# Clemapfel/kmer_index

Hardware: AMD Instinct MI355X
Metric: M queries/sec, DNA4 k=10 exact-match batch search, 1e8-bp text (higher is better)
Workload: dtype u32/u64

## Files before the change

kmer_index_amd/csrc/kmx_capi.hip:

```cpp
#include <hip/hip_runtime.h>

#include <algorithm>
#include <atomic>
#include <cstddef>
#include <cstdio>
#include <cstdlib>
#include <cstring>
#include <memory>
#include <mutex>
#include <string>
#include <system_error>
#include <thread>
#include <vector>

#include "kmx_approx.h"
#include "kmx_host.h"
#include "kmx_kernels.h"

namespace {

thread_local std::string g_err;

kmx_status fail(kmx_status st, const std::string& msg)
{
// ... 1331 lines not shown
    if (r && !r->parts.empty()) return fail(KMX_ERR_INVALID_ARGUMENT, "kmx_search_batch_device: the result handle belongs to a multi-device search");
    if (r && r->device != ix->device && r->device_bytes())
        return fail(KMX_ERR_INVALID_ARGUMENT, "kmx_search_batch_device: the result handle holds buffers on another device");
    if (!r) { r = take_result(ix); *inout = r; }
    else if (r->ctx.pending) { kmx_status fs = search_finish(r); if (fs != KMX_OK) return fs; }
    r->index = ix;
    r->device = ix->device;
    r->stream = s;
    (void)hipGetLastError();
    r->flags = flags;
    r->nq = nq;
    r->n_hits = r->n_exact = r->n_stitch = r->n_prefix = r->n_error = r->n_none = r->n_mask_words = 0;
    r->host_valid = r->host_masks_valid = false;
    r->small_valid = false;
    r->quiesced = false;
    if (!r->h_ctr) HIP_TRY(hipHostMalloc(reinterpret_cast<void**>(&r->h_ctr), KMX_CTR_COUNT * sizeof(unsigned long long), hipHostMallocDefault));
    HIP_TRY(r->hit_off.ensure((nq + 1) * 8));
    if (nq == 0) {
        HIP_TRY(hipMemsetAsync(r->hit_off.p, 0, 8, s));
        return KMX_OK;
    }
    HIP_TRY(r->src.ensure(nq * 8));
    HIP_TRY(r->cnt.ensure(nq * 4));
    HIP_TRY(r->c0.ensure(nq * 4));
    HIP_TRY(r->aux.ensure(nq * 8));
    HIP_TRY(r->key.ensure(nq * 8));
    HIP_TRY(r->p1.ensure(nq * 8));
    HIP_TRY(r->kind.ensure(nq));
    HIP_TRY(r->status.ensure(nq));
    HIP_TRY(r->stitch_list.ensure(nq * 4));
    HIP_TRY(r->prefix_list.ensure(nq * 4));
    HIP_TRY(r->short_list.ensure(nq * 4));
    HIP_TRY(r->bsum.ensure(std::max(kmx::scan_blocks(nq), kmx::lookup_blocks(nq, 4)) * 8));
    if (r->ctr.cap < 2 * KMX_CTR_COUNT * sizeof(unsigned long long)) {
        HIP_TRY(r->ctr.ensure(2 * KMX_CTR_COUNT * sizeof(unsigned long long)));
        HIP_TRY(hipMemsetAsync(r->ctr.p, 0, 2 * KMX_CTR_COUNT * sizeof(unsigned long long), s));
        r->ctr_phase = 0;
        r->ctr_clean = true;
    }
    kmx::QueryDesc d{r->src.as<uint64_t>(), r->cnt.as<uint32_t>(), r->c0.as<uint32_t>(), r->aux.as<uint64_t>(),
                     r->key.as<uint64_t>(), r->p1.as<uint64_t>(), r->kind.as<uint8_t>(), r->status.as<uint8_t>(),
                     r->stitch_list.as<uint32_t>(), r->prefix_list.as<uint32_t>(), r->short_list.as<uint32_t>(), nullptr};
    if (!r->ctr_clean) {
        HIP_TRY(hipMemsetAsync(r->ctr.p, 0, 2 * KMX_CTR_COUNT * sizeof(unsigned long long), s));
        r->ctr_clean = true;
    }
    r->ctr_phase ^= 1u;
    auto* ctr = r->ctr.as<unsigned long long>() + r->ctr_phase * KMX_CTR_COUNT;
    auto* ctr_next = r->ctr.as<unsigned long long>() + (r->ctr_phase ^ 1u) * KMX_CTR_COUNT;
    const KmxIndexDev* dix = header_for(ix, flags);

    static const int force_items = getenv("KMX_LOOKUP_ITEMS") ? atoi(getenv("KMX_LOOKUP_ITEMS")) : 0;
    const bool pairs = force_items ? force_items == -4 : r->last_had_pairs;
    const int items = force_items ? (force_items == 8 ? 8 : 4) : (!pairs && ix->tiny_cells) ? 8 : 4;
    const bool defer_long = r->last_had_long;
    const uint32_t lflags = (flags & ~KMX_SEARCH_INTERNAL_DEFER_LONG) | (defer_long ? KMX_SEARCH_INTERNAL_DEFER_LONG : 0u);
    timed(ix, K_LOOKUP, s, [&] {
        kmx::launch_lookup(s, items, pairs, dix, qr, qo, nq, d, ctr, r->bsum.as<uint64_t>(), lflags);
        if (defer_long) kmx::launch_lookup_long(s, dix, qr, qo, nq, d, ctr, flags);
    });
    const kmx::FillVariant fv = kmx::effective_fill_variant(ix->fill_variant, ix->rec32);
    const uint64_t tile = kmx::fill_tile(fv);
    const uint64_t tile_cap = r->tile_q.cap / 4;
    bool published = false;
    timed(ix, K_SCAN, s, [&] {
        published = kmx::launch_scan_tiles(s, d.cnt, nq, r->bsum.as<uint64_t>(), r->hit_off.as<uint64_t>(), ctr + KMX_CTR_TOTAL_HITS, tile,
                                           tile_cap >= 2 ? tile_cap - 1 : 0, tile_cap >= 2 ? r->tile_q.as<uint32_t>() : nullptr, items,
                                           kmx::CounterPub{ctr, ctr_next, r->h_ctr});
    });
    r->ctr_clean = published;
    const uint64_t spec_tiles = std::min<uint64_t>(tile_cap >= 2 ? tile_cap - 1 : 0, (r->out.cap / 4) / tile);
    const bool spec_fill = !(flags & KMX_SEARCH_COUNT_ONLY) && !r->last_had_stitch && spec_tiles > 0 && spec_tiles < 0x7FFFFFFFull;
    if (spec_fill)
        timed(ix, K_FILL, s, [&] {
            kmx::launch_fill(s, fv, ix->rec32, dix, ix->d_arena, r->hit_off.as<uint64_t>(), r->tile_q.as<uint32_t>(),
                             ctr + KMX_CTR_TOTAL_HITS, spec_tiles, d, r->out.as<uint32_t>());
        });
    if (!published) HIP_TRY(hipMemcpyAsync(r->h_ctr, ctr, KMX_CTR_COUNT * sizeof(unsigned long long), hipMemcpyDeviceToHost, s));
    r->ctx = SearchCtx{ix, qr, qo, s, tile_cap, spec_tiles, spec_fill, true};
    if (flags & KMX_SEARCH_ASYNC) {
        if (!r->done) HIP_TRY(hipEventCreateWithFlags(&r->done, hipEventDisableTiming));
        HIP_TRY(hipEventRecord(r->done, s));
        r->pool = ix->pool;
        std::lock_guard<std::mutex> lock(ix->pool->mu);
        ix->pool->pending.push_back(r);
        return KMX_OK;
    }
    return search_finish(r);
}

static kmx_status search_finish(kmx_result* r)
{
    if (!r->ctx.pending) return KMX_OK;
    r->ctx.pending = false;
    kmx_index* ix = r->ctx.ix;
    if (r->flags & KMX_SEARCH_ASYNC) {
        std::lock_guard<std::mutex> lock(ix->pool->mu);
        auto& pend = ix->pool->pending;
        pend.erase(std::remove(pend.begin(), pend.end(), r), pend.end());
    }
    const uint8_t* qr = r->ctx.qr;
// ... 1088 lines not shown
```

kmer_index_amd/csrc/kmx_kernels.h:

```cpp
#pragma once
#include <hip/hip_runtime.h>
#include <stdint.h>
#include "kmx_types.h"


namespace kmx {

struct QueryDesc {
    uint64_t* src;
    uint32_t* cnt;
    uint32_t* c0;
    uint64_t* aux;
    uint64_t* key;
    uint64_t* p1;
    uint8_t* kind;
    uint8_t* status;
    uint32_t* stitch_list;
    uint32_t* prefix_list;
    uint32_t* short_list;
    uint32_t* stitch_hits;
};

uint64_t lookup_blocks(uint64_t nq, int items);
void launch_lookup(hipStream_t s, int items, bool pairs, const KmxIndexDev* ix, const uint8_t* qranks, const uint64_t* qoff,
                   uint64_t nq, const QueryDesc& d, unsigned long long* ctr, uint64_t* block_hits, uint32_t flags);
void launch_lookup_long(hipStream_t s, const KmxIndexDev* ix, const uint8_t* qranks, const uint64_t* qoff, uint64_t nq, const QueryDesc& d,
                        unsigned long long* ctr, uint32_t flags);
void launch_validate(hipStream_t s, const KmxIndexDev* ix, const uint32_t* arena, const uint8_t* qranks, const uint64_t* qoff,
                     const QueryDesc& d, uint64_t n_stitch, uint64_t n_more, uint64_t n_tiny, const uint32_t* tiny_list, uint64_t n_short,
                     uint64_t* mask_words, bool direct);
void launch_small(hipStream_t s, const KmxIndexDev* ix, const uint32_t* arena, unsigned char* mailbox, const KmxSmallLayout& layout, uint32_t n_blocks,
                  const KmxSmallArgs& args, uint32_t nq_total, unsigned long long* xchg, uint32_t flags);
uint64_t scan_blocks(uint64_t n);
void launch_build_dir(hipStream_t s, const uint64_t* d_ukeys, uint64_t n_ukeys, uint32_t shift, uint32_t n_dir, uint32_t* d_dir);
void launch_build_cells(hipStream_t s, const uint32_t* d_offs, const uint32_t* d_region, uint64_t n_keys, uint32_t cell_shift,
                        uint32_t* d_cells, uint8_t* d_cnt8);

struct SparseTables {
    uint64_t* d_ukeys = nullptr;
    uint32_t* d_offs = nullptr;
    KmxSlot* d_slots = nullptr;
    uint64_t n_ukeys = 0;
    uint32_t log2cap = 0;
};
hipError_t sort_kmer_positions(hipStream_t s, const uint8_t* d_text, uint64_t n, uint32_t k, uint32_t sigma, uint32_t key_bits,
                               uint32_t* d_positions);
hipError_t build_sparse_element(hipStream_t s, const uint8_t* d_text, uint64_t n, uint32_t k, uint32_t sigma, uint32_t key_bits,
                                uint32_t* d_positions, SparseTables* out);
hipError_t sort_pairs_u64(hipStream_t s, uint64_t* keys_a, uint32_t* vals_a, uint64_t* keys_b, uint32_t* vals_b, uint64_t n, uint32_t key_bits,
                          bool* in_b);
void launch_scan(hipStream_t s, const uint32_t* in, uint64_t n, uint64_t* bsum, uint64_t* out,
                 unsigned long long* total_out);
struct FillVariant {
    int e;
    bool nt;
};
struct CounterPub {
    const unsigned long long* cur = nullptr;
    unsigned long long* next = nullptr;
    unsigned long long* host = nullptr;
};
bool launch_scan_tiles(hipStream_t s, const uint32_t* in, uint64_t n, uint64_t* bsum, uint64_t* out,
                       unsigned long long* total_out, uint64_t tile, uint64_t n_tiles_cap, uint32_t* tile_q, int lookup_items,
                       const CounterPub& pub = CounterPub());
FillVariant effective_fill_variant(const FillVariant& v, bool rec32);
uint64_t fill_tile(const FillVariant& v);
void launch_partition(hipStream_t s, const uint64_t* off, uint64_t nq, uint64_t tile, uint64_t n_tiles, uint32_t* tile_q);
void launch_fill(hipStream_t s, const FillVariant& v, bool rec32, const KmxIndexDev* ix, const uint32_t* arena, const uint64_t* hit_off,
                 const uint32_t* tile_q, const unsigned long long* total_dev, uint64_t n_tiles, const QueryDesc& d, uint32_t* out);
void launch_compact(hipStream_t s, const uint32_t* arena, const QueryDesc& d, uint64_t n_stitch,
                    const uint64_t* mask_words, const uint64_t* hit_off, uint32_t* out);
void launch_prefix_len(hipStream_t s, const QueryDesc& d, uint64_t n_prefix, const uint32_t* banded, uint32_t* plen);
void launch_build_phase1(hipStream_t s, const uint8_t* d_text, uint64_t n, uint32_t k, uint32_t sigma, uint64_t n_keys,
                         uint32_t* d_hist, uint64_t* d_scratch_u64, uint64_t* d_bsum, uint32_t* d_offs, uint32_t* d_cursor,
                         unsigned int* d_info, unsigned long long* d_total);
void launch_build_phase2(hipStream_t s, const uint8_t* d_text, uint64_t n, uint32_t k, uint32_t sigma, uint64_t n_keys,
                         const uint32_t* d_offs, uint32_t* d_hist, uint64_t* d_scratch_u64, uint64_t* d_bsum, uint32_t* d_cursor,
                         unsigned int* d_info, unsigned long long* d_total, uint32_t* d_region, uint32_t* d_aoffs, uint32_t a0,
                         int sort_mode, uint32_t* d_atab, uint32_t region_end);
void launch_bucket_sort_block(hipStream_t s, const uint32_t* d_offs, uint64_t n_keys, uint32_t* d_positions);
void launch_prefix_sort_small(hipStream_t s, const KmxIndexDev* ix, const uint64_t* qoff, const QueryDesc& d, uint64_t n_prefix,
                              const uint64_t* hit_off, const uint32_t* arena, uint32_t* out);
void launch_prefix_merge_small(hipStream_t s, const KmxIndexDev* ix, const uint64_t* qoff, const QueryDesc& d, uint64_t n_prefix,
                               const uint64_t* hit_off, const uint32_t* arena, uint32_t* out);
struct PrefixSplitRoom {
    void* splits; uint64_t cap_splits;
    void* tiles; uint64_t cap_tiles;
    uint32_t* counters; uint64_t cap_counters;
    uint32_t* scratch; uint64_t cap_scratch;
};
void launch_prefix_bands(hipStream_t s, const KmxIndexDev* ix, const uint64_t* qoff, const QueryDesc& d, uint64_t n_prefix, const uint64_t* hit_off,
                         const uint32_t* arena, uint32_t* banded, void* bands, uint64_t cap_bands, uint32_t* cuts, uint64_t cap_cuts,
                         unsigned long long* used, const PrefixSplitRoom& sr);
void launch_prefix_split(hipStream_t s, const PrefixSplitRoom& sr, const unsigned long long* used, const uint32_t* arena, uint32_t* banded, uint64_t n_text,
                         void* items, uint64_t cap_items, unsigned long long* n_other);
uint64_t prefix_split_bytes(int what);
uint64_t prefix_split_target();
// ... 19 lines not shown
```

kmer_index_amd/csrc/kmx_kernels.hip:

```cpp
#include <hip/hip_runtime.h>
#include <stdint.h>

#include <algorithm>
#include <atomic>
#include <type_traits>

#include "kmx_kernels.h"

#define KMX_BLOCK 256
#define KMX_WAVE 64
#define KMX_PSORT_PAIR_CAP 512
#ifndef KMX_PSORT_MULTIWAY_RUNS
#define KMX_PSORT_MULTIWAY_RUNS 4
#endif
#define KMX_PM_WAVE_EMAX (((KMX_PSORT_CAP + (KMX_WAVE - KMX_PSORT_MAX_RUNS / 2) - 1) / (KMX_WAVE - KMX_PSORT_MAX_RUNS / 2)) | 1)
#define KMX_PM_WAVE_PAD (KMX_PSORT_MAX_RUNS + KMX_PM_WAVE_EMAX + 5)
#define KMX_PM_TILE 4096
#define KMX_STAGE_CAP 1024
#define KMX_VGROUP 16
#define KMX_VGROUPS (KMX_WAVE / KMX_VGROUP)
#define KMX_VSLICES (64 / KMX_VGROUP)
#define KMX_VSTAGE (1024 / KMX_VGROUPS)
#define KMX_VCH 8

// ... 467 lines not shown
                const KMX_GLOBAL uint32_t* offs = as_global(el->offs);
                const uint32_t a = offs[h], e = offs[h + 1];
                r.src = el->arena_base + a; r.cnt = e - a;
            }
        }
        else if (el->atab) { r.src = el->arena_base + (pr[0] & ~31u); r.cnt = atab_count(pr[0], pr[1]); }
        else { r.src = el->arena_base + pr[0]; r.cnt = pr[1] - pr[0]; }
        return r;
    }
    const KMX_GLOBAL KmxSlot* slots = as_global(el->slots);
    const uint64_t mask = (uint64_t(1) << el->log2cap) - 1;
    uint64_t s = slot_hash_dev(h, el->log2cap);
    uint64_t key = uint64_t(pr[0]) | (uint64_t(pr[1]) << 32);
    uint32_t off = pr[2], c = pr[3];
    while (c != 0 && key != h) {
        s = (s + 1) & mask;
        const u64x2 raw = *(const KMX_GLOBAL u64x2*)(slots + s);
        key = raw.x; off = uint32_t(raw.y); c = uint32_t(raw.y >> 32);
    }
    if (c) { r.src = el->arena_base + off; r.cnt = c; }
    return r;
}

#define KMX_PLAN_LDS 256

#ifndef KMX_LOOKUP_OCC
#define KMX_LOOKUP_OCC 4
#endif
template <int ITEMS, bool PAIRS>
__global__ __launch_bounds__(KMX_BLOCK, PAIRS ? KMX_LOOKUP_OCC : (ITEMS > 4 ? 4 : 5)) void k_lookup(const KmxIndexDev* __restrict__ ix,
                                                      const uint8_t* __restrict__ qranks,
                                                      const uint64_t* __restrict__ qoff, uint64_t nq,
                                                      QueryDesc d, unsigned long long* __restrict__ ctr,
                                                      uint64_t* __restrict__ block_hits, uint32_t flags)
{
    __shared__ BlockCounters bc;
    __shared__ KmxElemDev elems_s[KMX_MAX_KS];
    __shared__ uint32_t plan_s[KMX_PLAN_LDS];
    static_assert(KMX_PLAN_LDS == KMX_BLOCK, "one planner entry per thread");
    if (threadIdx.x == 0) {
        bc.n_long = 0;
        bc.n_stitch = bc.n_stitch_tiny = bc.n_stitch_short = bc.n_resolved = bc.n_prefix = bc.n_prefix_big = bc.n_prefix_merge = bc.n_prefix_mid = bc.n_prefix_plain = bc.n_error = bc.n_none = bc.n_more = 0;
        bc.words = bc.pelems = bc.hits = 0;
        bc.max_runs = 0;
        unsigned int j = 0;
        while (j < 63 && ix->pw[j + 1] <= KMX_SUBK_FANOUT_LIMIT) ++j;
        bc.max_fan_exp = j;
        unsigned int small = ix->sigma < (1u << 24) ? 1u : 0u;
        for (uint32_t e = 0; e < ix->n_ks; ++e) {
            const uint64_t nk = ix->elems[e].n_keys;
            if (nk > (uint64_t(1) << 32) || nk / ix->sigma > (uint64_t(1) << 24)) small = 0;
        }
        bc.small_keys = small;
    }
    {
        const uint32_t n_words = ix->n_ks * uint32_t(sizeof(KmxElemDev) / 8);
        const uint64_t* __restrict__ srcw = reinterpret_cast<const uint64_t*>(ix->elems);
        uint64_t* dstw = reinterpret_cast<uint64_t*>(elems_s);
        for (uint32_t i = threadIdx.x; i < n_words; i += KMX_BLOCK) dstw[i] = srcw[i];
        plan_s[threadIdx.x] = threadIdx.x < ix->range ? ((const KMX_GLOBAL uint32_t*)ix->plan)[threadIdx.x] : 0u;
    }
    const uint8_t* __restrict__ qend = qranks + qoff[nq];
    __syncthreads();

    uint8_t kinds[ITEMS];
    unsigned int locs[ITEMS];
    unsigned long long locw[ITEMS];
// ... 246 lines not shown
#pragma unroll 1
    for (int it = 0; it < ITEMS; ++it) {
        if (done[it]) continue;
        const uint64_t q = (uint64_t(blockIdx.x) * ITEMS + it) * KMX_BLOCK + threadIdx.x;
        if (q >= nq) continue;
        const uint64_t b = qoff[q];
        const uint64_t m = qoff[q + 1] - b;
        if (m > 0 && m < range) {
            const KmxPlanEntry pe = plan_unpack(plan_effective(m < KMX_PLAN_LDS ? plan_s[m] : ((const KMX_GLOBAL uint32_t*)ix->plan)[m]));
            if (pe.scheme == KMX_SCHEME_SINGLE) {
                const uint32_t k = elems_s[pe.elem].k;
                if (m > uint64_t(k) * KMX_LONG_PARTS) {
                    const unsigned int slot = atomicAdd(&bc.n_long, 1u);
                    if (flags & KMX_SEARCH_INTERNAL_DEFER_LONG) {
                        kinds[it] = 0xFF;
                        locs[it] = slot;
                        continue;
                    }
                }
            }
        }
        LookupOut lo;
        lookup_query(ix, elems_s, qranks + b, m, qend, flags & ~KMX_SEARCH_INTERNAL_DEFER_LONG, lo);
        emit(it, q, lo.kind, lo.status, lo.src, lo.aux, lo.key, lo.p1, lo.cnt, lo.c0, lo.resolved);
    }

    if (my_resolved) atomicAdd(&bc.n_resolved, my_resolved);
    if (my_err) atomicAdd(&bc.n_error, my_err);
    if (my_none) atomicAdd(&bc.n_none, my_none);
    for (int off = 32; off > 0; off >>= 1) my_hits += __shfl_xor(my_hits, off);
    if (lane_id() == 0 && my_hits) atomicAdd(&bc.hits, (unsigned long long)my_hits);
    __syncthreads();
    if (threadIdx.x == 0) {
        if (block_hits) block_hits[blockIdx.x] = bc.hits;
        if (bc.n_stitch | bc.n_stitch_tiny | bc.n_stitch_short) {
            if (bc.n_stitch) bc.base_stitch = (unsigned int)atomicAdd(&ctr[KMX_CTR_STITCH], (unsigned long long)bc.n_stitch);
            if (bc.n_stitch_tiny) bc.base_stitch_tiny = (unsigned int)atomicAdd(&ctr[KMX_CTR_STITCH_TINY], (unsigned long long)bc.n_stitch_tiny);
            if (bc.n_stitch_short) bc.base_stitch_short = (unsigned int)atomicAdd(&ctr[KMX_CTR_STITCH_SHORT], (unsigned long long)bc.n_stitch_short);
            bc.base_words = atomicAdd(&ctr[KMX_CTR_MASK_WORDS], bc.words);
            if (bc.n_more) atomicAdd(&ctr[KMX_CTR_STITCH_MORE], (unsigned long long)bc.n_more);
        }
        if (bc.n_prefix) bc.base_prefix = (unsigned int)atomicAdd(&ctr[KMX_CTR_PREFIX], (unsigned long long)bc.n_prefix);
        if (bc.n_prefix_merge) atomicAdd(&ctr[KMX_CTR_PREFIX_MERGE], (unsigned long long)bc.n_prefix_merge);
        if (bc.n_prefix_mid) atomicAdd(&ctr[KMX_CTR_PREFIX_MID], (unsigned long long)bc.n_prefix_mid);
        if (bc.n_prefix_plain) atomicAdd(&ctr[KMX_CTR_PREFIX_PLAIN], (unsigned long long)bc.n_prefix_plain);
        if (bc.n_prefix_big) {
            bc.base_prefix_big = (unsigned int)atomicAdd(&ctr[KMX_CTR_PREFIX_BIG], (unsigned long long)bc.n_prefix_big);
            if (bc.pelems) atomicAdd(&ctr[KMX_CTR_PREFIX_ELEMS], bc.pelems);
            if (bc.max_runs) atomicMax(&ctr[KMX_CTR_MAX_RUNS], (unsigned long long)bc.max_runs);
        }
        if (bc.n_long) bc.base_long = (unsigned int)atomicAdd(&ctr[KMX_CTR_LONG], (unsigned long long)bc.n_long);
        if (bc.n_resolved) atomicAdd(&ctr[KMX_CTR_STITCH_RESOLVED], (unsigned long long)bc.n_resolved);
        if (bc.n_error) atomicAdd(&ctr[KMX_CTR_ERROR], (unsigned long long)bc.n_error);
        if (bc.n_none) atomicAdd(&ctr[KMX_CTR_NONE], (unsigned long long)bc.n_none);
    }
    __syncthreads();
#pragma unroll
    for (int it = 0; it < ITEMS; ++it) {
        const uint64_t q = (uint64_t(blockIdx.x) * ITEMS + it) * KMX_BLOCK + threadIdx.x;
        if (kinds[it] == 0xFF) {
            d.short_list[nq - 1 - (bc.base_long + locs[it])] = uint32_t(q);
        } else if (kinds[it] == KMX_KIND_STITCH) {
            d.aux[q] = bc.base_words + locw[it];
            if (locs[it] & 0x80000000u) d.stitch_list[nq - 1 - (bc.base_stitch_tiny + (locs[it] & 0x3FFFFFFFu))] = uint32_t(q);
            else if (locs[it] & 0x40000000u) d.short_list[bc.base_stitch_short + (locs[it] & 0x3FFFFFFFu)] = uint32_t(q);
            else d.stitch_list[bc.base_stitch + locs[it]] = uint32_t(q);
        } else if (kinds[it] == KMX_KIND_PREFIX && locs[it] != 0xFFFFFFFFu) {
// ... 1331 lines not shown
{
    const uint64_t base = uint64_t(blockIdx.x) * KMX_SCAN_TILE;
    uint64_t s = 0;
#pragma unroll
    for (int j = 0; j < KMX_SCAN_ITEMS; ++j) {
        uint64_t i = base + uint64_t(j) * KMX_BLOCK + threadIdx.x;
        if (i < n) s += in[i];
    }
    uint64_t total;
    block_exclusive_scan_u64(s, &total);
    if (threadIdx.x == 0) bsum[blockIdx.x] = total;
}

__global__ __launch_bounds__(KMX_BLOCK) void k_scan_spine(uint64_t* __restrict__ bsum, uint64_t nb,
                                                          unsigned long long* __restrict__ total_out)
{
    uint64_t running = 0;
    for (uint64_t base = 0; base < nb; base += KMX_BLOCK) {
        uint64_t i = base + threadIdx.x;
        uint64_t v = i < nb ? bsum[i] : 0;
        uint64_t total;
        uint64_t ex = block_exclusive_scan_u64(v, &total);
        if (i < nb) bsum[i] = running + ex;
        running += total;
    }
    if (threadIdx.x == 0) *total_out = running;
}

template <bool TILES, int SPINE>
__global__ __launch_bounds__(KMX_BLOCK) void k_scan_down(const uint32_t* __restrict__ in, uint64_t n,
                                                         const uint64_t* __restrict__ bsum,
                                                         uint64_t* __restrict__ out, uint64_t tile,
                                                         uint64_t n_tiles_cap, uint32_t* __restrict__ tile_q,
                                                         unsigned long long* __restrict__ total_out, uint64_t n_fine,
                                                         CounterPub pub, uint32_t fine_per_tile)
{
    static_assert(KMX_SCAN_TILE % (KMX_BLOCK * 8) == 0 && KMX_SCAN_TILE % (KMX_BLOCK * 4) == 0, "a scan tile is a whole number of lookup blocks");
    constexpr int ROWS = KMX_SCAN_ITEMS / 4;
    __shared__ uint64_t wave_sum[ROWS][KMX_BLOCK / KMX_WAVE];
    const uint32_t lane = lane_id(), w = threadIdx.x / KMX_WAVE;
    const uint64_t block_base = uint64_t(blockIdx.x) * KMX_SCAN_TILE;
    uint32_t v[ROWS][4];
    uint64_t inc[ROWS];
#pragma unroll
    for (int r = 0; r < ROWS; ++r) {
        const uint64_t i = block_base + uint64_t(r) * (KMX_BLOCK * 4) + uint64_t(threadIdx.x) * 4;
        if (i + 3 < n) {
            const uint4 t = *reinterpret_cast<const uint4*>(in + i);
            v[r][0] = t.x; v[r][1] = t.y; v[r][2] = t.z; v[r][3] = t.w;
        } else {
#pragma unroll
            for (int j = 0; j < 4; ++j) v[r][j] = i + j < n ? in[i + j] : 0u;
        }
        inc[r] = uint64_t(v[r][0]) + v[r][1] + v[r][2] + v[r][3];
    }
    uint64_t own[ROWS];
#pragma unroll
    for (int r = 0; r < ROWS; ++r) own[r] = inc[r];
    for (int off = 1; off < KMX_WAVE; off <<= 1) {
#pragma unroll
        for (int r = 0; r < ROWS; ++r) {
            const uint64_t t = __shfl_up(inc[r], off);
            if (lane >= uint32_t(off)) inc[r] += t;
        }
    }
    if (lane == KMX_WAVE - 1) {
#pragma unroll
        for (int r = 0; r < ROWS; ++r) wave_sum[r][w] = inc[r];
    }
    __syncthreads();
    uint64_t row_base;
    if constexpr (SPINE != 0) {
        __shared__ uint64_t part[KMX_BLOCK / KMX_WAVE];
        const uint64_t mine = SPINE == 2 ? uint64_t(blockIdx.x) * fine_per_tile : uint64_t(blockIdx.x);
        uint64_t acc = 0;
        for (uint64_t i = threadIdx.x; i < mine; i += KMX_BLOCK) acc += bsum[i];
        for (int off = 32; off > 0; off >>= 1) acc += __shfl_xor(acc, off);
        if (lane == 0) part[w] = acc;
        __syncthreads();
        row_base = 0;
#pragma unroll
        for (uint32_t i = 0; i < KMX_BLOCK / KMX_WAVE; ++i) row_base += part[i];
        if (blockIdx.x + 1 == gridDim.x && threadIdx.x == 0) {
            uint64_t own = 0;
            if constexpr (SPINE == 2) { for (uint64_t i = mine; i < n_fine; ++i) own += bsum[i]; }
            else own = bsum[blockIdx.x];
            *total_out = row_base + own;
            if (pub.host) {
#pragma unroll
                for (int c = 0; c < KMX_CTR_COUNT; ++c) {
                    pub.host[c] = c == KMX_CTR_TOTAL_HITS ? row_base + own : pub.cur[c];
                    pub.next[c] = 0;
                }
            }
        }
    } else {
        row_base = bsum[blockIdx.x];
    }
#pragma unroll
    for (int r = 0; r < ROWS; ++r) {
        uint64_t carry = 0, total = 0;
#pragma unroll
        for (uint32_t i = 0; i < KMX_BLOCK / KMX_WAVE; ++i) {
            const uint64_t sw = wave_sum[r][i];
            if (i < w) carry += sw;
            total += sw;
        }
        uint64_t ex = row_base + carry + inc[r] - own[r];
        row_base += total;
        const uint64_t i0 = block_base + uint64_t(r) * (KMX_BLOCK * 4) + uint64_t(threadIdx.x) * 4;
        uint64_t o[4];
#pragma unroll
        for (int j = 0; j < 4; ++j) {
            const uint64_t i = i0 + j;
            o[j] = ex;
            if constexpr (TILES) {
                if (i < n && v[r][j]) {
                    uint64_t t = (ex + tile - 1) / tile;
                    const uint64_t t_end = (ex + v[r][j] - 1) / tile;
                    for (; t <= t_end && t <= n_tiles_cap; ++t) tile_q[t] = uint32_t(i);
                }
            }
            ex += v[r][j];
            if (i + 1 == n) {
// ... 861 lines not shown
    __syncthreads();
    const KMX_LDS uint32_t* lb = (const KMX_LDS uint32_t*)buf;
    const uint32_t dg = min(tid * E, n_out);
    const uint32_t lo = merge_path_cut(lb, nA, lb + (nA + 1), nB, dg);
    uint32_t x[E];
    merge_chunk<int(E), false>(lb + lo, lb + (nA + 1 + dg - lo), nullptr, nullptr, E, x);
    __syncthreads();
#pragma unroll
    for (uint32_t j = 0; j < E; ++j)
        if (dg + j < n_out) buf[dg + j] = x[j];
    __syncthreads();
    for (uint32_t t = tid; t < n_out; t += KMX_BLOCK) dst[o0 + t] = buf[t];
}

static void allow_big_lds(const void* fn, size_t bytes, int which)
{
    static std::atomic<uint64_t> done[3] = {{0}, {0}, {0}};
    int dev = 0;
    if (hipGetDevice(&dev) != hipSuccess) { (void)hipGetLastError(); return; }
    const uint64_t bit = uint64_t(1) << (dev & 63);
    if (done[which].load(std::memory_order_acquire) & bit) return;
    (void)hipFuncSetAttribute(fn, hipFuncAttributeMaxDynamicSharedMemorySize, int(bytes));
    done[which].fetch_or(bit, std::memory_order_release);
}

static inline unsigned int blocks_for(uint64_t n, uint64_t per_block)
{
    uint64_t b = (n + per_block - 1) / per_block;
    return (unsigned int)(b ? b : 1);
}

uint64_t lookup_blocks(uint64_t nq, int items) { return blocks_for(nq, uint64_t(KMX_BLOCK) * uint64_t(items)); }

void launch_lookup(hipStream_t s, int items, bool pairs, const KmxIndexDev* ix, const uint8_t* qranks, const uint64_t* qoff,
                   uint64_t nq, const QueryDesc& d, unsigned long long* ctr, uint64_t* block_hits, uint32_t flags)
{
    const dim3 grid(blocks_for(nq, uint64_t(KMX_BLOCK) * uint64_t(items))), block(KMX_BLOCK);
    if (pairs) hipLaunchKernelGGL((k_lookup<4, true>), grid, block, 0, s, ix, qranks, qoff, nq, d, ctr, block_hits, flags);
    else if (items == 8) hipLaunchKernelGGL((k_lookup<8, false>), grid, block, 0, s, ix, qranks, qoff, nq, d, ctr, block_hits, flags);
    else hipLaunchKernelGGL((k_lookup<4, false>), grid, block, 0, s, ix, qranks, qoff, nq, d, ctr, block_hits, flags);
}

void launch_validate(hipStream_t s, const KmxIndexDev* ix, const uint32_t* arena, const uint8_t* qranks, const uint64_t* qoff,
                     const QueryDesc& d, uint64_t n_stitch, uint64_t n_more, uint64_t n_tiny, const uint32_t* tiny_list, uint64_t n_short,
                     uint64_t* mask_words, bool direct)
{
    if (n_tiny)
        hipLaunchKernelGGL(k_validate_tiny, dim3(blocks_for(n_tiny, KMX_BLOCK)), dim3(KMX_BLOCK), 0, s, ix, arena, qranks, qoff, d, tiny_list,
                           n_tiny, mask_words, direct && d.stitch_hits != nullptr);
    if (n_short) {
        const uint64_t swaves = (n_short + KMX_VGROUPS - 1) / KMX_VGROUPS;
        const unsigned int sblocks = (unsigned int)std::min<uint64_t>((swaves + 3) / 4, 256 * 32);
        hipLaunchKernelGGL(k_validate_short, dim3(sblocks ? sblocks : 1), dim3(KMX_BLOCK), 0, s, arena, d, n_short, mask_words);
    }
    if (!n_stitch) return;
    uint64_t waves = (n_stitch + KMX_VGROUPS - 1) / KMX_VGROUPS;
    unsigned int blocks = (unsigned int)std::min<uint64_t>((waves + 3) / 4, 256 * 32);
    const dim3 grid(blocks ? blocks : 1), block(KMX_BLOCK);
    if (n_more && !d.stitch_hits) {
        hipLaunchKernelGGL(k_validate<true>, grid, block, 0, s, ix, arena, qranks, qoff, d, n_stitch, mask_words);
        return;
    }
    hipLaunchKernelGGL(k_validate<false>, grid, block, 0, s, ix, arena, qranks, qoff, d, n_stitch, mask_words);
    if (n_more) {
        const uint64_t sw = (n_stitch + KMX_VWIDE_SCAN - 1) / KMX_VWIDE_SCAN;
        const unsigned int sblocks = (unsigned int)std::min<uint64_t>((sw + 3) / 4, 256 * 16);
        hipLaunchKernelGGL(k_validate_wide, dim3(sblocks ? sblocks : 1), dim3(KMX_VWIDE_BLOCK), 0, s, arena, d, n_stitch, mask_words);
        hipLaunchKernelGGL(k_validate_more_thread, dim3(blocks_for(n_stitch, KMX_BLOCK)), block, 0, s, ix, arena, qranks, qoff, d, n_stitch,
                           uint32_t(n_more >= KMX_VMORE_THREAD_MANY ? KMX_VMORE_THREAD_PARTS_MANY : KMX_VMORE_THREAD_PARTS), mask_words);
        hipLaunchKernelGGL(k_validate_more, grid, block, 0, s, ix, arena, qranks, qoff, d, n_stitch, mask_words);
        const uint64_t wwaves = (n_stitch + KMX_VWAVE_SCAN - 1) / KMX_VWAVE_SCAN;
        const unsigned int wblocks = (unsigned int)std::min<uint64_t>((wwaves + 3) / 4, 256 * 16);
        hipLaunchKernelGGL(k_validate_wave, dim3(wblocks ? wblocks : 1), block, 0, s, ix, arena, qranks, qoff, d, n_stitch, mask_words);
    }
}

uint64_t scan_blocks(uint64_t n) { return blocks_for(n, KMX_SCAN_TILE); }

#define KMX_SCAN_FUSED_SPINE_BLOCKS 8192

void launch_scan(hipStream_t s, const uint32_t* in, uint64_t n, uint64_t* bsum, uint64_t* out,
                 unsigned long long* total_out)
{
    const unsigned int nb = blocks_for(n, KMX_SCAN_TILE);
    hipLaunchKernelGGL(k_scan_reduce, dim3(nb), dim3(KMX_BLOCK), 0, s, in, n, bsum);
    if (nb <= KMX_SCAN_FUSED_SPINE_BLOCKS) {
        hipLaunchKernelGGL((k_scan_down<false, 1>), dim3(nb), dim3(KMX_BLOCK), 0, s, in, n, bsum, out, uint64_t(1), uint64_t(0),
                           (uint32_t*)nullptr, total_out, uint64_t(0), CounterPub(), 0u);
        return;
    }
    hipLaunchKernelGGL(k_scan_spine, dim3(1), dim3(KMX_BLOCK), 0, s, bsum, uint64_t(nb), total_out);
    hipLaunchKernelGGL((k_scan_down<false, 0>), dim3(nb), dim3(KMX_BLOCK), 0, s, in, n, bsum, out, uint64_t(1), uint64_t(0),
                       (uint32_t*)nullptr, total_out, uint64_t(0), CounterPub(), 0u);
}

bool launch_scan_tiles(hipStream_t s, const uint32_t* in, uint64_t n, uint64_t* bsum, uint64_t* out,
                       unsigned long long* total_out, uint64_t tile, uint64_t n_tiles_cap, uint32_t* tile_q, int lookup_items,
                       const CounterPub& pub)
{
    const unsigned int nb = blocks_for(n, KMX_SCAN_TILE);
    const bool lookup_sums = lookup_items != 0;
    if (lookup_sums && nb <= KMX_SCAN_FUSED_SPINE_BLOCKS) {
        const uint64_t n_fine = lookup_blocks(n, lookup_items);
        const uint32_t fine = uint32_t(KMX_SCAN_TILE / (KMX_BLOCK * lookup_items));
        if (tile_q)
            hipLaunchKernelGGL((k_scan_down<true, 2>), dim3(nb), dim3(KMX_BLOCK), 0, s, in, n, bsum, out, tile, n_tiles_cap, tile_q, total_out, n_fine, pub, fine);
        else
            hipLaunchKernelGGL((k_scan_down<false, 2>), dim3(nb), dim3(KMX_BLOCK), 0, s, in, n, bsum, out, uint64_t(1), uint64_t(0),
                               (uint32_t*)nullptr, total_out, n_fine, pub, fine);
        return pub.host != nullptr;
    }
    if (!tile_q) { launch_scan(s, in, n, bsum, out, total_out); return false; }
    hipLaunchKernelGGL(k_scan_reduce, dim3(nb), dim3(KMX_BLOCK), 0, s, in, n, bsum);
    if (nb <= KMX_SCAN_FUSED_SPINE_BLOCKS) {
        hipLaunchKernelGGL((k_scan_down<true, 1>), dim3(nb), dim3(KMX_BLOCK), 0, s, in, n, bsum, out, tile, n_tiles_cap, tile_q, total_out, uint64_t(0), CounterPub(), 0u);
        return false;
    }
    hipLaunchKernelGGL(k_scan_spine, dim3(1), dim3(KMX_BLOCK), 0, s, bsum, uint64_t(nb), total_out);
    hipLaunchKernelGGL((k_scan_down<true, 0>), dim3(nb), dim3(KMX_BLOCK), 0, s, in, n, bsum, out, tile, n_tiles_cap, tile_q, total_out, uint64_t(0), CounterPub(), 0u);
    return false;
}

uint64_t fill_tile(const FillVariant& v) { return uint64_t(KMX_BLOCK) * v.e; }

void launch_partition(hipStream_t s, const uint64_t* off, uint64_t nq, uint64_t tile, uint64_t n_tiles, uint32_t* tile_q)
{
    hipLaunchKernelGGL(k_partition, dim3(blocks_for(n_tiles + 1, KMX_BLOCK)), dim3(KMX_BLOCK), 0, s, off, nq, tile, n_tiles, tile_q);
}

FillVariant effective_fill_variant(const FillVariant& v, bool rec32)
{
    FillVariant e = v;
    if (!rec32) e.e = 8;
    if (e.e != 4 && e.e != 8 && e.e != 12 && e.e != 16) e.e = 12;
    return e;
}

void launch_fill(hipStream_t s, const FillVariant& v0, bool rec32, const KmxIndexDev* ix, const uint32_t* arena, const uint64_t* hit_off,
                 const uint32_t* tile_q, const unsigned long long* total, uint64_t n_tiles, const QueryDesc& d, uint32_t* out)
{
    const FillVariant v = effective_fill_variant(v0, rec32);
    const dim3 grid((unsigned int)n_tiles), block(KMX_BLOCK);
    if (!rec32) {
        if (v.nt) hipLaunchKernelGGL((k_fill<8, true, uint64_t>), grid, block, 0, s, ix, arena, hit_off, tile_q, total, d, out);
        else hipLaunchKernelGGL((k_fill<8, false, uint64_t>), grid, block, 0, s, ix, arena, hit_off, tile_q, total, d, out);
        return;
    }
#define KMX_FILL_CASE(E_, NT_)                                                                                          \
    if (v.e == E_ && v.nt == NT_) {                                                                                     \
        hipLaunchKernelGGL((k_fill<E_, NT_, uint32_t>), grid, block, 0, s, ix, arena, hit_off, tile_q, total, d, out);   \
        return;                                                                                                         \
    }
// ... 1326 lines not shown
```

kmer_index_amd/csrc/kmx_types.h:

```cpp
#pragma once
#include <stdint.h>
#include "../../include/kmx.h"

#define KMX_MAX_LEVELS 3
#define KMX_DEFAULT_PREFIX_LEVELS 2

struct KmxSlot {
    uint64_t key;
    uint32_t off;
    uint32_t cnt;
};

struct KmxElemDev {
    uint32_t k;
    uint32_t table_kind;
    uint32_t log2cap;
    uint32_t n_ukeys;
    uint64_t n_keys;
    uint64_t arena_base;
    uint64_t npos;
    const uint32_t* offs;
    const KmxSlot* slots;
    const uint64_t* ukeys;
    const uint32_t* atab;
// ... 93 lines not shown
    L.off_words = L.off_kinds + nq;
    L.off_pos = L.off_words + blocks * KMX_SMALL_WORDS * 8;
    L.bytes = L.off_pos + blocks * KMX_SMALL_POS * 4;
    L.pad = 0;
    return L;
}

enum {
    KMX_CTR_STITCH = 1,
    KMX_CTR_PREFIX = 2,
    KMX_CTR_ERROR = 3,
    KMX_CTR_MASK_WORDS = 4,
    KMX_CTR_PREFIX_ELEMS = 5,
    KMX_CTR_MAX_RUNS = 6,
    KMX_CTR_TOTAL_HITS = 7,
    KMX_CTR_NONE = 8,
    KMX_CTR_PREFIX_TOTAL = 9,
    KMX_CTR_STITCH_MORE = 10,
    KMX_CTR_PREFIX_BIG = 11,
    KMX_CTR_STITCH_TINY = 12,
    KMX_CTR_STITCH_RESOLVED = 13,
    KMX_CTR_PREFIX_MERGE = 14,
    KMX_CTR_PREFIX_MID = 15,
    KMX_CTR_PREFIX_PLAIN = 0,
    KMX_CTR_STITCH_SHORT = 16,
    KMX_CTR_LONG = 17,
    KMX_CTR_PSB_MERGE = 18,
    KMX_CTR_PSB_OTHER = 19,
    KMX_CTR_PSB_BANDS = 20,
    KMX_CTR_PSB_CUTS = 21,
    KMX_CTR_PSB_SPLITS = 22,
    KMX_CTR_COUNT = 28
};
#define KMX_LONG_PARTS 256
#define KMX_SEARCH_INTERNAL_DEFER_LONG 0x80000000u
```

Measured before the change: 7095.

## Add coarse per-group hit sums so fused scan spine avoids long prefix loops

The lookup kernel now atomically adds each block's hit count into a coarse per-64-block bucket. The fused scan downsweep then builds each tile's base from the coarse sums plus at most one group of fine sums, instead of summing all preceding fine block sums. The grand total is taken from the last block's own wave sums, and the next phase's coarse buffer is zeroed inside the scan. This replaces an O(blocks) per-tile prefix read with a two-level sum, at the cost of extra atomics in lookup and double-buffered coarse storage.

Measured after the change: 7070. Within noise of the previous version (-0.4%).

```diff
diff --git a/kmer_index_amd/csrc/kmx_capi.hip b/kmer_index_amd/csrc/kmx_capi.hip
--- a/kmer_index_amd/csrc/kmx_capi.hip
+++ b/kmer_index_amd/csrc/kmx_capi.hip
@@ -1387,9 +1387,10 @@
     HIP_TRY(r->prefix_list.ensure(nq * 4));
     HIP_TRY(r->short_list.ensure(nq * 4));
     HIP_TRY(r->bsum.ensure(std::max(kmx::scan_blocks(nq), kmx::lookup_blocks(nq, 4)) * 8));
-    if (r->ctr.cap < 2 * KMX_CTR_COUNT * sizeof(unsigned long long)) {
-        HIP_TRY(r->ctr.ensure(2 * KMX_CTR_COUNT * sizeof(unsigned long long)));
-        HIP_TRY(hipMemsetAsync(r->ctr.p, 0, 2 * KMX_CTR_COUNT * sizeof(unsigned long long), s));
+    const size_t ctr_bytes = 2 * (KMX_CTR_COUNT + KMX_LOOKUP_COARSE_CAP) * sizeof(unsigned long long);
+    if (r->ctr.cap < ctr_bytes) {
+        HIP_TRY(r->ctr.ensure(ctr_bytes));
+        HIP_TRY(hipMemsetAsync(r->ctr.p, 0, ctr_bytes, s));
         r->ctr_phase = 0;
         r->ctr_clean = true;
     }
@@ -1397,12 +1398,14 @@
                      r->key.as<uint64_t>(), r->p1.as<uint64_t>(), r->kind.as<uint8_t>(), r->status.as<uint8_t>(),
                      r->stitch_list.as<uint32_t>(), r->prefix_list.as<uint32_t>(), r->short_list.as<uint32_t>(), nullptr};
     if (!r->ctr_clean) {
-        HIP_TRY(hipMemsetAsync(r->ctr.p, 0, 2 * KMX_CTR_COUNT * sizeof(unsigned long long), s));
+        HIP_TRY(hipMemsetAsync(r->ctr.p, 0, ctr_bytes, s));
         r->ctr_clean = true;
     }
     r->ctr_phase ^= 1u;
     auto* ctr = r->ctr.as<unsigned long long>() + r->ctr_phase * KMX_CTR_COUNT;
     auto* ctr_next = r->ctr.as<unsigned long long>() + (r->ctr_phase ^ 1u) * KMX_CTR_COUNT;
+    uint64_t* coarse = r->ctr.as<uint64_t>() + 2 * KMX_CTR_COUNT + r->ctr_phase * KMX_LOOKUP_COARSE_CAP;
+    uint64_t* coarse_next = r->ctr.as<uint64_t>() + 2 * KMX_CTR_COUNT + (r->ctr_phase ^ 1u) * KMX_LOOKUP_COARSE_CAP;
     const KmxIndexDev* dix = header_for(ix, flags);
 
     static const int force_items = getenv("KMX_LOOKUP_ITEMS") ? atoi(getenv("KMX_LOOKUP_ITEMS")) : 0;
@@ -1411,7 +1414,7 @@
     const bool defer_long = r->last_had_long;
     const uint32_t lflags = (flags & ~KMX_SEARCH_INTERNAL_DEFER_LONG) | (defer_long ? KMX_SEARCH_INTERNAL_DEFER_LONG : 0u);
     timed(ix, K_LOOKUP, s, [&] {
-        kmx::launch_lookup(s, items, pairs, dix, qr, qo, nq, d, ctr, r->bsum.as<uint64_t>(), lflags);
+        kmx::launch_lookup(s, items, pairs, dix, qr, qo, nq, d, ctr, r->bsum.as<uint64_t>(), coarse, lflags);
         if (defer_long) kmx::launch_lookup_long(s, dix, qr, qo, nq, d, ctr, flags);
     });
     const kmx::FillVariant fv = kmx::effective_fill_variant(ix->fill_variant, ix->rec32);
@@ -1421,7 +1424,7 @@
     timed(ix, K_SCAN, s, [&] {
         published = kmx::launch_scan_tiles(s, d.cnt, nq, r->bsum.as<uint64_t>(), r->hit_off.as<uint64_t>(), ctr + KMX_CTR_TOTAL_HITS, tile,
                                            tile_cap >= 2 ? tile_cap - 1 : 0, tile_cap >= 2 ? r->tile_q.as<uint32_t>() : nullptr, items,
-                                           kmx::CounterPub{ctr, ctr_next, r->h_ctr});
+                                           kmx::CoarseSums{coarse, coarse_next}, kmx::CounterPub{ctr, ctr_next, r->h_ctr});
     });
     r->ctr_clean = published;
     const uint64_t spec_tiles = std::min<uint64_t>(tile_cap >= 2 ? tile_cap - 1 : 0, (r->out.cap / 4) / tile);
diff --git a/kmer_index_amd/csrc/kmx_kernels.h b/kmer_index_amd/csrc/kmx_kernels.h
--- a/kmer_index_amd/csrc/kmx_kernels.h
+++ b/kmer_index_amd/csrc/kmx_kernels.h
@@ -23,7 +23,7 @@
 
 uint64_t lookup_blocks(uint64_t nq, int items);
 void launch_lookup(hipStream_t s, int items, bool pairs, const KmxIndexDev* ix, const uint8_t* qranks, const uint64_t* qoff,
-                   uint64_t nq, const QueryDesc& d, unsigned long long* ctr, uint64_t* block_hits, uint32_t flags);
+                   uint64_t nq, const QueryDesc& d, unsigned long long* ctr, uint64_t* block_hits, uint64_t* coarse_hits, uint32_t flags);
 void launch_lookup_long(hipStream_t s, const KmxIndexDev* ix, const uint8_t* qranks, const uint64_t* qoff, uint64_t nq, const QueryDesc& d,
                         unsigned long long* ctr, uint32_t flags);
 void launch_validate(hipStream_t s, const KmxIndexDev* ix, const uint32_t* arena, const uint8_t* qranks, const uint64_t* qoff,
@@ -60,9 +60,13 @@
     unsigned long long* next = nullptr;
     unsigned long long* host = nullptr;
 };
+struct CoarseSums {
+    const uint64_t* cur = nullptr;
+    uint64_t* next = nullptr;
+};
 bool launch_scan_tiles(hipStream_t s, const uint32_t* in, uint64_t n, uint64_t* bsum, uint64_t* out,
                        unsigned long long* total_out, uint64_t tile, uint64_t n_tiles_cap, uint32_t* tile_q, int lookup_items,
-                       const CounterPub& pub = CounterPub());
+                       const CoarseSums& cs = CoarseSums(), const CounterPub& pub = CounterPub());
 FillVariant effective_fill_variant(const FillVariant& v, bool rec32);
 uint64_t fill_tile(const FillVariant& v);
 void launch_partition(hipStream_t s, const uint64_t* off, uint64_t nq, uint64_t tile, uint64_t n_tiles, uint32_t* tile_q);
diff --git a/kmer_index_amd/csrc/kmx_kernels.hip b/kmer_index_amd/csrc/kmx_kernels.hip
--- a/kmer_index_amd/csrc/kmx_kernels.hip
+++ b/kmer_index_amd/csrc/kmx_kernels.hip
@@ -523,7 +523,7 @@
                                                       const uint8_t* __restrict__ qranks,
                                                       const uint64_t* __restrict__ qoff, uint64_t nq,
                                                       QueryDesc d, unsigned long long* __restrict__ ctr,
-                                                      uint64_t* __restrict__ block_hits, uint32_t flags)
+                                                      uint64_t* __restrict__ block_hits, uint64_t* __restrict__ coarse_hits, uint32_t flags)
 {
     __shared__ BlockCounters bc;
     __shared__ KmxElemDev elems_s[KMX_MAX_KS];
@@ -836,7 +836,10 @@
     if (lane_id() == 0 && my_hits) atomicAdd(&bc.hits, (unsigned long long)my_hits);
     __syncthreads();
     if (threadIdx.x == 0) {
-        if (block_hits) block_hits[blockIdx.x] = bc.hits;
+        if (block_hits) {
+            block_hits[blockIdx.x] = bc.hits;
+            if (coarse_hits && bc.hits) atomicAdd(reinterpret_cast<unsigned long long*>(coarse_hits) + blockIdx.x / KMX_LOOKUP_GROUP, bc.hits);
+        }
         if (bc.n_stitch | bc.n_stitch_tiny | bc.n_stitch_short) {
             if (bc.n_stitch) bc.base_stitch = (unsigned int)atomicAdd(&ctr[KMX_CTR_STITCH], (unsigned long long)bc.n_stitch);
             if (bc.n_stitch_tiny) bc.base_stitch_tiny = (unsigned int)atomicAdd(&ctr[KMX_CTR_STITCH_TINY], (unsigned long long)bc.n_stitch_tiny);
@@ -2234,10 +2237,22 @@
                                                          const uint64_t* __restrict__ bsum,
                                                          uint64_t* __restrict__ out, uint64_t tile,
                                                          uint64_t n_tiles_cap, uint32_t* __restrict__ tile_q,
-                                                         unsigned long long* __restrict__ total_out, uint64_t n_fine,
+                                                         unsigned long long* __restrict__ total_out, CoarseSums cs,
                                                          CounterPub pub, uint32_t fine_per_tile)
 {
     static_assert(KMX_SCAN_TILE % (KMX_BLOCK * 8) == 0 && KMX_SCAN_TILE % (KMX_BLOCK * 4) == 0, "a scan tile is a whole number of lookup blocks");
+    static_assert(KMX_LOOKUP_GROUP <= KMX_BLOCK, "the fine sums of a group: one per thread");
+    uint64_t acc = 0;
+    if constexpr (SPINE == 2) {
+        const uint64_t mine = uint64_t(blockIdx.x) * fine_per_tile;
+        const uint64_t g = mine / KMX_LOOKUP_GROUP;
+        const uint64_t f = g * KMX_LOOKUP_GROUP + threadIdx.x;
+        if (f < mine) acc = bsum[f];
+        for (uint64_t i = threadIdx.x; i < g; i += KMX_BLOCK) acc += cs.cur[i];
+        if (cs.next) {
+            for (uint64_t i = uint64_t(blockIdx.x) * KMX_BLOCK + threadIdx.x; i < KMX_LOOKUP_COARSE_CAP; i += uint64_t(gridDim.x) * KMX_BLOCK) cs.next[i] = 0;
+        }
+    }
     constexpr int ROWS = KMX_SCAN_ITEMS / 4;
     __shared__ uint64_t wave_sum[ROWS][KMX_BLOCK / KMX_WAVE];
     const uint32_t lane = lane_id(), w = threadIdx.x / KMX_WAVE;
@@ -2274,9 +2289,9 @@
     uint64_t row_base;
     if constexpr (SPINE != 0) {
         __shared__ uint64_t part[KMX_BLOCK / KMX_WAVE];
-        const uint64_t mine = SPINE == 2 ? uint64_t(blockIdx.x) * fine_per_tile : uint64_t(blockIdx.x);
-        uint64_t acc = 0;
-        for (uint64_t i = threadIdx.x; i < mine; i += KMX_BLOCK) acc += bsum[i];
+        if constexpr (SPINE == 1) {
+            for (uint64_t i = threadIdx.x; i < blockIdx.x; i += KMX_BLOCK) acc += bsum[i];
+        }
         for (int off = 32; off > 0; off >>= 1) acc += __shfl_xor(acc, off);
         if (lane == 0) part[w] = acc;
         __syncthreads();
@@ -2284,14 +2299,16 @@
 #pragma unroll
         for (uint32_t i = 0; i < KMX_BLOCK / KMX_WAVE; ++i) row_base += part[i];
         if (blockIdx.x + 1 == gridDim.x && threadIdx.x == 0) {
-            uint64_t own = 0;
-            if constexpr (SPINE == 2) { for (uint64_t i = mine; i < n_fine; ++i) own += bsum[i]; }
-            else own = bsum[blockIdx.x];
-            *total_out = row_base + own;
+            uint64_t grand = row_base;
+#pragma unroll
+            for (int r = 0; r < ROWS; ++r)
+#pragma unroll
+                for (uint32_t i = 0; i < KMX_BLOCK / KMX_WAVE; ++i) grand += wave_sum[r][i];
+            *total_out = grand;
             if (pub.host) {
 #pragma unroll
                 for (int c = 0; c < KMX_CTR_COUNT; ++c) {
-                    pub.host[c] = c == KMX_CTR_TOTAL_HITS ? row_base + own : pub.cur[c];
+                    pub.host[c] = c == KMX_CTR_TOTAL_HITS ? grand : pub.cur[c];
                     pub.next[c] = 0;
                 }
             }
@@ -3219,13 +3236,19 @@
 
 uint64_t lookup_blocks(uint64_t nq, int items) { return blocks_for(nq, uint64_t(KMX_BLOCK) * uint64_t(items)); }
 
+#define KMX_SCAN_FUSED_SPINE_BLOCKS 8192
+static_assert(uint64_t(KMX_SCAN_FUSED_SPINE_BLOCKS) * (KMX_SCAN_TILE / (KMX_BLOCK * 4)) <= uint64_t(KMX_LOOKUP_GROUP) * KMX_LOOKUP_COARSE_CAP,
+              "a coarse sum for every group of k_lookup blocks of a batch the fused downsweep takes");
+static inline bool lookup_sums_fused(uint64_t nq) { return blocks_for(nq, KMX_SCAN_TILE) <= KMX_SCAN_FUSED_SPINE_BLOCKS; }
+
 void launch_lookup(hipStream_t s, int items, bool pairs, const KmxIndexDev* ix, const uint8_t* qranks, const uint64_t* qoff,
-                   uint64_t nq, const QueryDesc& d, unsigned long long* ctr, uint64_t* block_hits, uint32_t flags)
+                   uint64_t nq, const QueryDesc& d, unsigned long long* ctr, uint64_t* block_hits, uint64_t* coarse_hits, uint32_t flags)
 {
     const dim3 grid(blocks_for(nq, uint64_t(KMX_BLOCK) * uint64_t(items))), block(KMX_BLOCK);
-    if (pairs) hipLaunchKernelGGL((k_lookup<4, true>), grid, block, 0, s, ix, qranks, qoff, nq, d, ctr, block_hits, flags);
-    else if (items == 8) hipLaunchKernelGGL((k_lookup<8, false>), grid, block, 0, s, ix, qranks, qoff, nq, d, ctr, block_hits, flags);
-    else hipLaunchKernelGGL((k_lookup<4, false>), grid, block, 0, s, ix, qranks, qoff, nq, d, ctr, block_hits, flags);
+    if (!lookup_sums_fused(nq)) coarse_hits = nullptr;
+    if (pairs) hipLaunchKernelGGL((k_lookup<4, true>), grid, block, 0, s, ix, qranks, qoff, nq, d, ctr, block_hits, coarse_hits, flags);
+    else if (items == 8) hipLaunchKernelGGL((k_lookup<8, false>), grid, block, 0, s, ix, qranks, qoff, nq, d, ctr, block_hits, coarse_hits, flags);
+    else hipLaunchKernelGGL((k_lookup<4, false>), grid, block, 0, s, ix, qranks, qoff, nq, d, ctr, block_hits, coarse_hits, flags);
 }
 
 void launch_validate(hipStream_t s, const KmxIndexDev* ix, const uint32_t* arena, const uint8_t* qranks, const uint64_t* qoff,
@@ -3264,8 +3287,6 @@
 
 uint64_t scan_blocks(uint64_t n) { return blocks_for(n, KMX_SCAN_TILE); }
 
-#define KMX_SCAN_FUSED_SPINE_BLOCKS 8192
-
 void launch_scan(hipStream_t s, const uint32_t* in, uint64_t n, uint64_t* bsum, uint64_t* out,
                  unsigned long long* total_out)
 {
@@ -3273,38 +3294,37 @@
     hipLaunchKernelGGL(k_scan_reduce, dim3(nb), dim3(KMX_BLOCK), 0, s, in, n, bsum);
     if (nb <= KMX_SCAN_FUSED_SPINE_BLOCKS) {
         hipLaunchKernelGGL((k_scan_down<false, 1>), dim3(nb), dim3(KMX_BLOCK), 0, s, in, n, bsum, out, uint64_t(1), uint64_t(0),
-                           (uint32_t*)nullptr, total_out, uint64_t(0), CounterPub(), 0u);
+                           (uint32_t*)nullptr, total_out, CoarseSums(), CounterPub(), 0u);
         return;
     }
     hipLaunchKernelGGL(k_scan_spine, dim3(1), dim3(KMX_BLOCK), 0, s, bsum, uint64_t(nb), total_out);
     hipLaunchKernelGGL((k_scan_down<false, 0>), dim3(nb), dim3(KMX_BLOCK), 0, s, in, n, bsum, out, uint64_t(1), uint64_t(0),
-                       (uint32_t*)nullptr, total_out, uint64_t(0), CounterPub(), 0u);
+                       (uint32_t*)nullptr, total_out, CoarseSums(), CounterPub(), 0u);
 }
 
 bool launch_scan_tiles(hipStream_t s, const uint32_t* in, uint64_t n, uint64_t* bsum, uint64_t* out,
                        unsigned long long* total_out, uint64_t tile, uint64_t n_tiles_cap, uint32_t* tile_q, int lookup_items,
-                       const CounterPub& pub)
+                       const CoarseSums& cs, const CounterPub& pub)
 {
     const unsigned int nb = blocks_for(n, KMX_SCAN_TILE);
-    const bool lookup_sums = lookup_items != 0;
-    if (lookup_sums && nb <= KMX_SCAN_FUSED_SPINE_BLOCKS) {
-        const uint64_t n_fine = lookup_blocks(n, lookup_items);
+    const bool lookup_sums = lookup_items != 0 && cs.cur != nullptr;
+    if (lookup_sums && lookup_sums_fused(n)) {
         const uint32_t fine = uint32_t(KMX_SCAN_TILE / (KMX_BLOCK * lookup_items));
         if (tile_q)
-            hipLaunchKernelGGL((k_scan_down<true, 2>), dim3(nb), dim3(KMX_BLOCK), 0, s, in, n, bsum, out, tile, n_tiles_cap, tile_q, total_out, n_fine, pub, fine);
+            hipLaunchKernelGGL((k_scan_down<true, 2>), dim3(nb), dim3(KMX_BLOCK), 0, s, in, n, bsum, out, tile, n_tiles_cap, tile_q, total_out, cs, pub, fine);
         else
             hipLaunchKernelGGL((k_scan_down<false, 2>), dim3(nb), dim3(KMX_BLOCK), 0, s, in, n, bsum, out, uint64_t(1), uint64_t(0),
-                               (uint32_t*)nullptr, total_out, n_fine, pub, fine);
-        return pub.host != nullptr;
+                               (uint32_t*)nullptr, total_out, cs, pub, fine);
+        return pub.host != nullptr && cs.next != nullptr;
     }
     if (!tile_q) { launch_scan(s, in, n, bsum, out, total_out); return false; }
     hipLaunchKernelGGL(k_scan_reduce, dim3(nb), dim3(KMX_BLOCK), 0, s, in, n, bsum);
     if (nb <= KMX_SCAN_FUSED_SPINE_BLOCKS) {
-        hipLaunchKernelGGL((k_scan_down<true, 1>), dim3(nb), dim3(KMX_BLOCK), 0, s, in, n, bsum, out, tile, n_tiles_cap, tile_q, total_out, uint64_t(0), CounterPub(), 0u);
+        hipLaunchKernelGGL((k_scan_down<true, 1>), dim3(nb), dim3(KMX_BLOCK), 0, s, in, n, bsum, out, tile, n_tiles_cap, tile_q, total_out, CoarseSums(), CounterPub(), 0u);
         return false;
     }
     hipLaunchKernelGGL(k_scan_spine, dim3(1), dim3(KMX_BLOCK), 0, s, bsum, uint64_t(nb), total_out);
-    hipLaunchKernelGGL((k_scan_down<true, 0>), dim3(nb), dim3(KMX_BLOCK), 0, s, in, n, bsum, out, tile, n_tiles_cap, tile_q, total_out, uint64_t(0), CounterPub(), 0u);
+    hipLaunchKernelGGL((k_scan_down<true, 0>), dim3(nb), dim3(KMX_BLOCK), 0, s, in, n, bsum, out, tile, n_tiles_cap, tile_q, total_out, CoarseSums(), CounterPub(), 0u);
     return false;
 }
 
diff --git a/kmer_index_amd/csrc/kmx_types.h b/kmer_index_amd/csrc/kmx_types.h
--- a/kmer_index_amd/csrc/kmx_types.h
+++ b/kmer_index_amd/csrc/kmx_types.h
@@ -149,5 +149,7 @@
     KMX_CTR_PSB_SPLITS = 22,
     KMX_CTR_COUNT = 28
 };
+#define KMX_LOOKUP_GROUP 64
+#define KMX_LOOKUP_COARSE_CAP 512
 #define KMX_LONG_PARTS 256
 #define KMX_SEARCH_INTERNAL_DEFER_LONG 0x80000000u
```
